# Zaggy1024/RaytracerCore

Measured on AMD Instinct MI355X. Metric: Mrays/sec (primary+secondary) and samples/sec at 1080p, Cornell box, higher is better.
Workload: dtype f32; 1 GPU; bounce.txt camera 0 1920x1080 x 256 spp per GPU per step; traversal=brute, recursion=10, kernel_build=scene-specialised (hiprtc)

## Files before the change

### raytracercore_amd/csrc/kernels_path.hip

```cpp
#include "../../include/rtcore_rng.h"
#include "rt_kernels.h"
#ifdef RT_SCENE_CONST
#include "rt_scene_const.h"
#endif

namespace rtc {
namespace {

struct V3 {
    float x, y, z;
};
__device__ __forceinline__ V3 v3(float x, float y, float z) { return V3{x, y, z}; }
__device__ __forceinline__ V3 xyz(float4 a) { return V3{a.x, a.y, a.z}; }
__device__ __forceinline__ V3 operator+(V3 a, V3 b) { return {a.x + b.x, a.y + b.y, a.z + b.z}; }
__device__ __forceinline__ V3 operator-(V3 a, V3 b) { return {a.x - b.x, a.y - b.y, a.z - b.z}; }
__device__ __forceinline__ V3 operator*(V3 a, float s) { return {a.x * s, a.y * s, a.z * s}; }
__device__ __forceinline__ V3 operator*(V3 a, V3 b) { return {a.x * b.x, a.y * b.y, a.z * b.z}; }
__device__ __forceinline__ V3 operator-(V3 a) { return {-a.x, -a.y, -a.z}; }
__device__ __forceinline__ float dot(V3 a, V3 b) { return fmaf(a.x, b.x, fmaf(a.y, b.y, a.z * b.z)); }
__device__ __forceinline__ bool known_zero(float c)
{
#if defined(RT_SCENE_CONST)
    return __builtin_constant_p(c) && c == 0.0f;
#else
// ... 815 lines not shown
            col = xyz(M.specular) + xyz(M.diffuse) + emis;
            return 1;
        }
        if (S.bounce >= s.recursion) {
            rec->type = RT_BOUNCE_RECURSION_COMPLETE;
            col = S.tint * emis;
            return 1;
        }
    }

    const float shin = M.shininess;
    float z = 1.0f, sz = 0.0f;
    if (!(s.facts & FACT_INF_SHININESS) || !(__builtin_isinf(shin) && shin > 0.0f)) {
        const float a = __builtin_amdgcn_logf(next_u(S.rng)) * M.inv_shininess;
        z = __builtin_amdgcn_exp2f(a);
        sz = fsqrt(one_minus_exp2_2a<!SLOT>(a, z));
    }
    const Frame fr = make_frame(nrm);
    const V3 rough = horizon(fr, nrm, z, sz, next_u(S.rng));

    const float diff_lum = M.diffuse.w, emis_lum = M.emission.w;
    float spec_lum = M.specular.w, refr_lum = M.refraction.w;
    const float cs = -dot(rough, S.d);
    if constexpr (REC) rec->cos_in = cs;
    float cos_out = 0.0f, ior_ratio = 0.0f;
    const bool some_lum = SLOT ? ((refr_lum > 0.0f) | (spec_lum > 0.0f))
                               : ((__float_as_int(refr_lum) > 0) | (__float_as_int(spec_lum) > 0));
    if ((s.facts & FACT_IOR) && some_lum && M.ior != 0.0f &&
        cs >= 0.0f) {
        ior_ratio = inside ? M.eta_exit : M.eta_enter;
        const float sin_out = ior_ratio * fsqrt(1.0f - cs * cs);
        if (sin_out >= 1.0f) {
            refr_lum = 0.0f;
            if constexpr (REC) rec->fresnel = 1.0f;
        } else {
            cos_out = fsqrt(1.0f - sin_out * sin_out);
            const float ra = fmaf(-ior_ratio, cos_out, cs), rb = fmaf(ior_ratio, cos_out, cs);
            const float pa = fmaf(ior_ratio, cs, -cos_out), pb = fmaf(ior_ratio, cs, cos_out);
            const float ratio = (ra * ra * pb * pb + pa * pa * rb * rb) * rcp(rb * rb * pb * pb) * 0.5f;
            spec_lum *= ratio;
            refr_lum *= 1.0f - ratio;
            if constexpr (REC) rec->fresnel = ratio;
        }
    } else {
        refr_lum = 0.0f;
    }
    const float total = diff_lum + spec_lum + refr_lum + emis_lum;
    if (total <= 0.0f) {
        if constexpr (REC) rec->type = RT_BOUNCE_PURE_BLACK;
        col = S.tint * emis;
        return 1;
    }
    float ray_rand = next_u(S.rng) * total;
    const bool transmit = refr_lum != 0.0f && (ray_rand -= refr_lum) <= 0.0f;
    const bool specular = !transmit && spec_lum != 0.0f && (ray_rand -= spec_lum) <= 0.0f;
    const bool diffuse = !transmit && !specular && diff_lum != 0.0f && (ray_rand -= diff_lum) <= 0.0f;
    if (!(transmit | specular | diffuse)) {
        if constexpr (REC) rec->type = RT_BOUNCE_EMISSION;
        col = S.tint * emis;
        return 1;
    }
    if constexpr (REC) rec->type = transmit ? RT_BOUNCE_TRANSMITTED : specular ? RT_BOUNCE_SPECULAR : RT_BOUNCE_DIFFUSE;
    V3 out_dir, new_tint;
    if (diffuse) {
        const float dz = acos_turn2(next_u(S.rng));
        const float ds = fsqrt(fmaxf(0.0f, 1.0f - dz * dz));
        out_dir = horizon(fr, nrm, dz, ds, next_u(S.rng));
        new_tint = xyz(M.diffuse);
    } else {
        const float al = transmit ? ior_ratio : 1.0f;
        const float be = transmit ? cs * ior_ratio - cos_out : 2.0f * cs;
        out_dir = madd(rough, be, S.d * al);
        if (specular && !(dot(out_dir, nrm) > 0.0f)) {
            if constexpr (REC) rec->type = RT_BOUNCE_SPECULAR_FAIL;
            col = S.tint * emis;
            return 1;
        }
        new_tint = transmit ? (inside ? v3(1.0f, 1.0f, 1.0f) : xyz(M.refraction)) : xyz(M.specular);
    }
    S.o = pos;
    S.d = out_dir * (renormalise_at<SLOT>(s, S.bounce + 1) ? fmaf(-0.5f, dot(out_dir, out_dir), 1.5f) : 1.0f);
    S.prev = b.sg >> 1;
    if (VN && s.n_vn > 0 && kind == RT_PRIM_TRIANGLE && (fl & F_HASNORMALS)) {
        bool gin2;
        if (!__builtin_isnan(S.d.x + S.d.y + S.d.z) && vn_rehit_test(prims_d[id], (double)bu, (double)bv, S.d, gin2) &&
            ((fl & F_TWOSIDED) || !(gin2 ^ ((fl & F_INVERT) != 0)))) {
            const bool front = dot(out_dir, nrm) > 0.0f;
            if (front ? (gin2 == gin) : (gin2 != gin))
                S.prev = -2 - ((b.sg & ~1) | (int)gin2);
        }
    }
    S.tint = S.tint * (new_tint * (SLOT ? fmaxf(total, 1.0f) : vmax1(total)));
    S.bounce++;
    return 0;
}

#ifndef RT_PATH_WAVES
#define RT_PATH_WAVES 7
#endif
#ifndef RT_GROUPED_WAVES
#define RT_GROUPED_WAVES 7
#endif
#ifndef RT_WIDE_STACK
#define RT_WIDE_STACK 16
#endif
#ifndef RT_SPEC_PRIMS
#define RT_SPEC_PRIMS 2
#endif
#ifndef RT_BVH_WAVES
#define RT_BVH_WAVES 7
#endif
#ifndef RT_BVH2_WAVES
#define RT_BVH2_WAVES 6
#endif

struct ShadeRecs {
    const PrimF* prims;
    const MatF* mats;
    const XformF* xfs;
};
template <bool LDS, class SceneT>
__device__ __forceinline__ ShadeRecs stage_scene(const SceneT& s, const PrimF* prims_g, const MatF* mats_g,
                                                 const XformF* xf, float4* lds_scene)
{
    if (!LDS) return ShadeRecs{prims_g, mats_g, xf};
    const int n_p = s.n_slots * (int)(sizeof(PrimF) / 16), n_m = s.n_mats * (int)(sizeof(MatF) / 16),
              n_x = s.n_xf * (int)(sizeof(XformF) / 16);
    const float4* gp = reinterpret_cast<const float4*>(prims_g);
    const float4* gm = reinterpret_cast<const float4*>(mats_g);
    const float4* gx = reinterpret_cast<const float4*>(xf);
    for (int i = threadIdx.x; i < n_p; i += blockDim.x) lds_scene[i] = gp[i];
    for (int i = threadIdx.x; i < n_m; i += blockDim.x) lds_scene[n_p + i] = gm[i];
    for (int i = threadIdx.x; i < n_x; i += blockDim.x) lds_scene[n_p + n_m + i] = gx[i];
    __syncthreads();
    return ShadeRecs{reinterpret_cast<const PrimF*>(lds_scene), reinterpret_cast<const MatF*>(lds_scene + n_p),
                     reinterpret_cast<const XformF*>(lds_scene + n_p + n_m)};
}

__device__ __forceinline__ int scene_lds_float4s(const PathScene& s)
{
    return s.n_slots * (int)(sizeof(PrimF) / 16) + s.n_mats * (int)(sizeof(MatF) / 16) +
           s.n_xf * (int)(sizeof(XformF) / 16);
}

struct Lane {
    bool active, item_open, live;
    unsigned item;
    int fx, fy, s_next;
    rt_key2 pkey;
    float ar, ag, ab;
    unsigned cnt;
    unsigned pool_next, pool_end;
    unsigned split_j;
};

__device__ __forceinline__ void lane_init(Lane& L)
{
    L.active = true;
    L.item_open = L.live = false;
    L.item = 0;
    L.fx = L.fy = L.s_next = 0;
    L.pkey = rt_key2{0u, 0u};
    L.ar = L.ag = L.ab = 0.0f;
    L.cnt = 0;
    L.pool_next = L.pool_end = 0;
    L.split_j = 0;
}

__device__ __forceinline__ unsigned lanes_below(unsigned long long m)
{
    return __builtin_amdgcn_mbcnt_hi((unsigned)(m >> 32), __builtin_amdgcn_mbcnt_lo((unsigned)m, 0u));
}
template <bool TABLE = false, class ParT>
__device__ __forceinline__ void item_pixel(unsigned item, const ParT& p, int& px, int& py, int& c, int& fx, int& fy)
{
    const unsigned q = item & 63u, t = item >> 6;
    c = (int)(t & (unsigned)(p.n_chunks - 1));
    unsigned by, bx;
    const unsigned blk = t >> p.log2_chunks;
    if (TABLE && p.cull != nullptr) {
        const unsigned v = p.cull[kCullTable + blk];
        bx = v & 0xFFFFu;
        by = v >> 16;
    } else if (p.magic_bx != 0) {
        by = __umulhi(blk, p.magic_bx);
        bx = blk - by * (unsigned)p.blocks_x;
    } else {
        divmod(blk, (unsigned)p.blocks_x, p.inv_blocks_x, by, bx);
    }
    px = (int)bx * 8 + (int)(q & 7);
    py = (int)by * 8 + (int)(q >> 3);
    fx = p.x0 + px;
    fy = p.y0 + py;
    if (p.band > 0) {
        unsigned bq, br;
        if (p.band_log2 >= 0) {
            bq = (unsigned)py >> p.band_log2;
            br = (unsigned)py & (unsigned)(p.band - 1);
        } else {
            divmod((unsigned)py, (unsigned)p.band, p.inv_band, bq, br);
        }
        fy = p.y0 + ((int)bq * p.band_stride + p.band_offset) * p.band + (int)br;
    }
}

struct QueryRay {
    V3 o, d;
    bool valid;
};
__device__ __forceinline__ QueryRay load_query_ray(const double2* __restrict__ rays, unsigned i)
{
    const double2 r0 = rays[4 * (size_t)i], r1 = rays[4 * (size_t)i + 1], r2 = rays[4 * (size_t)i + 2],
                  r3 = rays[4 * (size_t)i + 3];
    QueryRay q;
    q.o = v3((float)r0.x, (float)r0.y, (float)r1.x);
    q.d = v3((float)r2.x, (float)r2.y, (float)r3.x);
    const float inf = __builtin_huge_valf();
    const bool finite = (fabsf(q.o.x) < inf) & (fabsf(q.o.y) < inf) & (fabsf(q.o.z) < inf) & (fabsf(q.d.x) < inf) &
                        (fabsf(q.d.y) < inf) & (fabsf(q.d.z) < inf) & (fabs(r1.y) < __builtin_huge_val()) &
                        (fabs(r3.y) < __builtin_huge_val());
    q.valid = finite & ((q.d.x != 0.0f) | (q.d.y != 0.0f) | (q.d.z != 0.0f));
    return q;
}

template <class ParT>
__device__ __forceinline__ unsigned item_ray(unsigned item, const ParT& p)
{
    return ((item >> (6 + p.log2_chunks)) << 6) | (item & 63u);
}

template <class ParT>
__device__ __forceinline__ void list_pixel(unsigned pix, const ParT& p, int& fx, int& fy)
{
    unsigned q, r;
    divmod(pix, (unsigned)p.scene.width, p.inv_frame_w, q, r);
    fx = (int)r;
    fy = (int)q;
}

template <bool NT, class ParT>
__device__ __forceinline__ int item_sample(const Lane& L, const ParT& p)
{
    if (!NT) return L.s_next;
    const int c = (int)((L.item >> 6) & (unsigned)(p.n_chunks - 1));
    return c * p.chunk + (int)(L.cnt & 0xFFu) + (int)((L.cnt >> 8) & 0xFFu);
}
template <bool NT, int SRC, bool ROWS, class ParT, class CamT>
__device__ __forceinline__ bool start_rows_on(const ParT& p, [[maybe_unused]] const CamT& cam)
{
    if constexpr (NT || SRC != ITEMS_TILE || !ROWS) {
        return false;
    } else {
#ifdef RT_SCENE_CONST
        if (!cam_frustum(cam) || cam_dof(cam)) return false;
#endif
        return p.starts != nullptr;
    }
}
typedef float row_f4 __attribute__((ext_vector_type(4)));
#ifdef __HIP_DEVICE_COMPILE__
typedef __attribute__((address_space(1))) row_f4 row_g4;
typedef __attribute__((address_space(1))) unsigned char row_g1;
#else
typedef row_f4 row_g4;
typedef unsigned char row_g1;
#endif
template <class ParT>
__device__ __forceinline__ unsigned start_row_offset(const ParT& p, unsigned r, int lane)
{
    const unsigned wave = blockIdx.x * 4u + (unsigned)__builtin_amdgcn_readfirstlane((int)(threadIdx.x >> 6));
    return (((wave * (unsigned)p.start_rows + r) << 6) | (unsigned)lane) * 16u;
}

template <bool NT, int SRC = ITEMS_TILE, bool ROWS = false, class ParT, class SceneT, class CamT>
__device__ __forceinline__ void refill(Lane& L, Sample& S, const ParT& p, const SceneT& s, const CamT& cam, int lane,
                                      unsigned total)
{
    const bool need = L.active && !L.live && (!L.item_open || L.cnt < 65536u);
    if (need && L.item_open) {
        const float4 part = make_float4(L.ar, L.ag, L.ab, __uint_as_float((L.cnt & 0xFFu) | ((L.cnt & 0xFF00u) << 8)));
        if (NT) {
            typedef float nt_f4 __attribute__((ext_vector_type(4)));
            const nt_f4 v = {part.x, part.y, part.z, part.w};
            __builtin_nontemporal_store(v, reinterpret_cast<nt_f4*>(&p.partial[L.item]));
        } else {
            p.partial[L.item] = part;
        }
        L.item_open = false;
        L.ar = L.ag = L.ab = 0.0f;
    }
    const unsigned long long m = __ballot(need);
    if (m) {
        unsigned k = (unsigned)__popcll(m);
        const unsigned avail = L.pool_end - L.pool_next;
        unsigned fresh = 0, fresh_len = (unsigned)p.pool;
        bool draw = k > avail;
        if (!NT && draw && k < (unsigned)p.batch && __ballot(L.active && !need) != 0ull) {
            draw = false;
            k = avail;
        }
        if (draw) {
            const bool linear = p.linear != 0;
            unsigned got = linear ? total : (unsigned)p.n_split << 28;
            if (lane == 0) {
                if (p.n_split <= 1) {
                    const unsigned f = atomicAdd(p.counter, 1u);
                    if (f < p.split_tickets[0]) got = linear ? f * (unsigned)p.pool : f;
                } else {
                    const unsigned g0 = blockIdx.x & (unsigned)(p.n_split - 1);
                    for (; L.split_j < (unsigned)p.n_split; L.split_j++) {
                        const unsigned g = (g0 + L.split_j) & (unsigned)(p.n_split - 1);
                        const unsigned f = atomicAdd(p.counter + kSplitStride * g, 1u);
                        if (f < p.split_tickets[g]) {
                            got = linear ? p.split_start[g] + f * (unsigned)p.pool : f | g << 28;
                            break;
                        }
                    }
                }
            }
            got = __builtin_amdgcn_readfirstlane(got);
            fresh = linear ? got : total;
            if (!linear && (got >> 28) < (unsigned)p.n_split)
                ticket_items(p, got >> 28, got & 0xFFFFFFFu, fresh, fresh_len);
        }
        if (need) {
            const unsigned r = NT ? lanes_below(m) : (unsigned)__popcll(m & ((1ull << lane) - 1ull));
            L.item = r < avail ? L.pool_next + r : fresh + (r - avail);
            if (r >= k) {
            } else if (L.item >= total) {
                L.active = false;
            } else if constexpr (SRC == ITEMS_PIXELS) {
                const unsigned li = item_ray(L.item, p);
                const int s0 = (int)((L.item >> 6) & (unsigned)(p.n_chunks - 1)) * p.chunk;
                if (li < p.n_rays && s0 < p.spp) {
                    const unsigned pix = p.pixel_list[li];
                    if (pix < p.n_frame_px) {
                        L.item_open = true;
                        if (!NT) L.s_next = s0;
                        L.cnt = (unsigned)(min(p.spp, s0 + p.chunk) - s0) << 16;
                        if (!NT) {
                            list_pixel(pix, p, L.fx, L.fy);
                            if (p.pkeys) L.pkey = p.pkeys[pix];
                            else L.pkey = rt_rng_pixel_key(p.seed_key, (unsigned long long)pix);
                        }
                    }
                }
            } else if constexpr (SRC == ITEMS_RAYS) {
                const unsigned ri = item_ray(L.item, p);
                const int s0 = (int)((L.item >> 6) & (unsigned)(p.n_chunks - 1)) * p.chunk;
                if (ri < p.n_rays && s0 < p.spp) {
                    L.item_open = true;
                    if (!NT) L.s_next = s0;
                    L.cnt = (unsigned)(min(p.spp, s0 + p.chunk) - s0) << 16;
                    if (!NT) {
                        L.fx = (int)ri;
                        L.pkey = rt_rng_pixel_key(p.seed_key, p.stream_base + (unsigned long long)ri);
                    }
                }
            } else {
                int px, py, c, fx, fy;
                item_pixel<!NT>(L.item, p, px, py, c, fx, fy);
                if (px < p.w && py < p.h && c * p.chunk < p.spp) {
                    L.item_open = true;
                    const int s0 = c * p.chunk;
                    if (!NT) L.s_next = s0;
                    L.cnt = (unsigned)(min(p.spp, s0 + p.chunk) - s0) << 16;
                    if (!NT) {
                        L.fx = fx;
                        L.fy = fy;
                    }
                    const unsigned long long pix = (unsigned long long)fy * (unsigned long long)p.scene.width +
                                                   (unsigned long long)fx;
                    if (!NT && p.pkeys) L.pkey = p.pkeys[pix];
                    else if (!NT) L.pkey = rt_rng_pixel_key(p.seed_key, pix);
                }
            }
        }
        if (draw) {
            L.pool_next = fresh + (k - avail);
            L.pool_end = fresh + fresh_len;
        } else {
            L.pool_next += k;
        }
        if (k != 0 && start_rows_on<NT, SRC, ROWS>(p, cam)) {
            const unsigned n = need && L.item_open ? L.cnt >> 16 : 0u;
            row_g1* const rows = (row_g1*)(unsigned long long)p.starts;
            for (unsigned j = 0; j < (unsigned)p.start_rows; j++) {
                if (j < n) {
                    S.rng = rt_rng_from_pixel_key(L.pkey, p.sample_base + (unsigned long long)(L.s_next + (int)j));
                    float sx, sy;
                    sample_point<true>(L.fx, L.fy, S, sx, sy);
                    S.d = camera_ray(cam, sx, sy).d;
                    const row_f4 v = {S.d.x, S.d.y, S.d.z, __uint_as_float(S.rng.x)};
                    *(row_g4*)(rows + start_row_offset(p, j, lane)) = v;
                }
            }
        }
    }
    if constexpr (SRC == ITEMS_RAYS) {
        if (L.active && L.item_open && !L.live && L.cnt >= 65536u) {
            const unsigned ri = NT ? item_ray(L.item, p) : (unsigned)L.fx;
            if (NT) L.pkey = rt_rng_pixel_key(p.seed_key, p.stream_base + (unsigned long long)ri);
            const QueryRay q = load_query_ray(p.ray_list, ri);
            if (q.valid) {
                S.rng = rt_rng_from_pixel_key(L.pkey, p.sample_base + (unsigned long long)item_sample<NT>(L, p));
                (void)rt_rng_next24(&S.rng);
                (void)rt_rng_next24(&S.rng);
                S.o = q.o;
                S.d = q.d;
                S.tint = v3(1.0f, 1.0f, 1.0f);
                S.bounce = 0;
                S.prev = -1;
                L.live = true;
            } else {
                const unsigned left = L.cnt >> 16;
                L.cnt = (L.cnt & 0xFFFFu) + (left << 8);
                if (!NT) L.s_next += (int)left;
            }
        }
        return;
    }
    if (L.active && L.item_open && !L.live && L.cnt >= 65536u) {
        if (start_rows_on<NT, SRC, ROWS>(p, cam)) {
            const unsigned r = (L.cnt & 0xFFu) + ((L.cnt >> 8) & 0xFFu);
            const row_g1* const rows = (const row_g1*)(unsigned long long)p.starts;
            const row_f4 v = *(const row_g4*)(rows + start_row_offset(p, r, lane));
            const V3 d = v3(v.x, v.y, v.z);
            S.rng.x = __float_as_uint(v.w);
            S.o = madd(d, cam.image_plane, xyz(cam.position));
            S.d = d;
            S.tint = v3(1.0f, 1.0f, 1.0f);
            S.bounce = 0;
            S.prev = -1;
            L.live = true;
            return;
        }
        int fx = L.fx, fy = L.fy;
        if (NT && SRC == ITEMS_PIXELS) {
            const unsigned pix = p.pixel_list[item_ray(L.item, p)];
            list_pixel(pix, p, fx, fy);
            L.pkey = rt_rng_pixel_key(p.seed_key, (unsigned long long)pix);
        } else if (NT) {
            int px, py, c;
            item_pixel(L.item, p, px, py, c, fx, fy);
            L.pkey = rt_rng_pixel_key(p.seed_key, (unsigned long long)fy * (unsigned long long)p.scene.width +
                                                      (unsigned long long)fx);
        }
        S.rng = rt_rng_from_pixel_key(L.pkey, p.sample_base + (unsigned long long)item_sample<NT>(L, p));
        start_sample<!NT>(cam, fx, fy, S);
        L.live = true;
    }
}

template <bool VN, bool PIN = false, bool SLOT = false, bool REC = false, class SceneT, class VnP, class TestP, class ParT>
__device__ __forceinline__ void bounce(Lane& L, Sample& S, const SceneT& s, const ShadeRecs& R, VnP vnormals, TestP tests,
                                       const PrimD* prims_d, const Best& b, [[maybe_unused]] const ParT& p)
{
    V3 col;
    [[maybe_unused]] BounceRec rec;
    [[maybe_unused]] const V3 ro = S.o, rd = S.d, rtint = S.tint;
    [[maybe_unused]] const int rbounce = S.bounce;
    [[maybe_unused]] unsigned rsample = 0;
    if constexpr (REC) {
        if (p.rec_rays) {
            int px, py, c, fx, fy;
            item_pixel(L.item, p, px, py, c, fx, fy);
            rsample = ((unsigned)py * (unsigned)p.w + (unsigned)px) * (unsigned)p.spp + (unsigned)item_sample<SLOT>(L, p);
        }
    }
    const int r = shade<VN, PIN, SLOT, REC>(s, R.prims, R.mats, R.xfs, vnormals, tests, prims_d, b, S, col, &rec);
    if constexpr (REC) {
        const unsigned slot = rsample * (unsigned)(s.recursion + 1) + (unsigned)rbounce;
        if (p.rec_rays && slot < p.rec_max && rbounce <= s.recursion) {
            float4* q = p.rec_rays + (size_t)kRecRows * slot;
            q[0] = make_float4(__int_as_float(rec.prim_id), __int_as_float(rec.type), __int_as_float(rec.inside), rec.distance);
            q[1] = make_float4(rec.fresnel, rec.cos_in, __int_as_float(rbounce), 0.0f);
            q[2] = make_float4(rec.pos.x, rec.pos.y, rec.pos.z, rec.nrm.x);
            q[3] = make_float4(rec.nrm.y, rec.nrm.z, ro.x, ro.y);
            q[4] = make_float4(ro.z, rd.x, rd.y, rd.z);
            q[5] = make_float4(rtint.x, rtint.y, rtint.z, 0.0f);
            if (r != 0)
                p.rec_samples[rsample] = r == 1 ? make_float4(0.0f + col.x, 0.0f + col.y, 0.0f + col.z, __int_as_float(rbounce + 1))
                                                : make_float4(-1.0f, -1.0f, -1.0f, __int_as_float(rbounce + 1));
        }
    }
    if (r != 0) {
        const bool hit = r == 1;
        L.ar += hit ? col.x : 0.0f;
        L.ag += hit ? col.y : 0.0f;
        L.ab += hit ? col.z : 0.0f;
        L.cnt += hit ? 1u - 65536u : 256u - 65536u;
        if (!SLOT) L.s_next++;
        L.live = false;
        if (!SLOT) {
            asm volatile("" : "=v"(S.o.x), "=v"(S.o.y), "=v"(S.o.z), "=v"(S.d.x), "=v"(S.d.y), "=v"(S.d.z),
                         "=v"(S.tint.x), "=v"(S.tint.y), "=v"(S.tint.z), "=v"(S.bounce), "=v"(S.prev),
                         "=v"(S.rng.x));
        }
    }
}

template <bool STATS, class ParT>
__device__ __forceinline__ void flush_counts(unsigned long long wave_rays, const Counters& cnt, const ParT& p,
                                             int lane)
{
    if (lane == 0) atomicAdd(p.rays, wave_rays);
    if (STATS) {
        unsigned long long a = cnt.nodes, t = cnt.tris, q = cnt.sphs;
        for (int off = 32; off > 0; off >>= 1) {
            a += __shfl_down(a, off);
            t += __shfl_down(t, off);
            q += __shfl_down(q, off);
        }
        if (lane == 0) {
            atomicAdd(p.stats + 0, a);
            atomicAdd(p.stats + 1, t);
            atomicAdd(p.stats + 2, q);
            atomicAdd(p.stats + 3, cnt.cyc_start);
            atomicAdd(p.stats + 4, cnt.cyc_trace);
            atomicAdd(p.stats + 5, cnt.cyc_shade);
            atomicAdd(p.stats + 6, cnt.iters);
        }
        unsigned long long mx = cnt.max_steps, ov = cnt.ovf_pushes, ms = cnt.max_sp, ot = cnt.outer;
        for (int off = 32; off > 0; off >>= 1) {
            mx = max(mx, (unsigned long long)__shfl_down(mx, off));
            ov += __shfl_down(ov, off);
            ms = max(ms, (unsigned long long)__shfl_down(ms, off));
            ot += __shfl_down(ot, off);
        }
        if (lane == 0) {
            atomicMax(p.stats + 7, mx);
            atomicAdd(p.stats + 8, ov);
            atomicMax(p.stats + 9, ms);
            atomicAdd(p.stats + 10, ot);
        }
    }
}

#ifdef __HIP_DEVICE_COMPILE__
#define RT_AS_CONST __attribute__((address_space(4)))
#else
#define RT_AS_CONST
#endif
typedef RT_AS_CONST const CameraF CameraC;
typedef RT_AS_CONST const PathParams ParamsC;

template <bool CULL, bool LDS, bool STATS, bool VN, int SRC = ITEMS_TILE>
__device__ __forceinline__ void path_body(const CameraF* __restrict__ camp, const PathParams* __restrict__ pp)
{
    const ParamsC& P0 = *(const ParamsC*)pp;
    extern __shared__ float4 lds_scene[];
    const ShadeRecs R = stage_scene<LDS>(P0.scene, P0.prims, P0.mats, P0.xf, lds_scene);
    const int lane = threadIdx.x & 63;
    const unsigned total = (unsigned)P0.n_chunks * (unsigned)P0.n_pad;
    Lane L;
    lane_init(L);
    Sample S;
    S.prev = -1;
    S.bounce = 0;
    Counters cnt{};
    unsigned long long wave_rays = 0;
    const unsigned long long bound_off = P0.scene_bound != 0 ? 0ull : ~0ull;

    while (true) {
        unsigned long long t0 = 0, t1 = 0, t2 = 0;
        if (STATS) t0 = __builtin_readcyclecounter();
        const CameraC* cp = (const CameraC*)camp;
        asm volatile("" : "+s"(cp));
        const ParamsC* pq = (const ParamsC*)pp;
        asm volatile("" : "+s"(pq));
#ifdef RT_SCENE_CONST
        const PathScene& sc = *(const PathScene*)kSceneW;
#else
        const auto& sc = pq->scene;
#endif
#if defined(RT_SCENE_CONST) && RT_SCENE_CONST_CAMERA
        refill<false, ITEMS_TILE, !STATS && !VN>(L, S, *pq, sc, *(const CameraF*)kCameraW, lane, total);
#else
        refill<false, SRC, !STATS && !VN>(L, S, *pq, sc, *cp, lane, total);
#endif
        if (!__any(L.active)) break;
        if (STATS) t1 = __builtin_readcyclecounter();
        wave_rays += (unsigned)__popcll(__ballot(L.live));
        if (L.live) {
#ifdef RT_SCENE_CONST
            const auto tests = (const TestRec*)kTestsW;
            const auto rects = (const RectRec*)kRectsW;
            const auto frames = (const FrameRec*)kFramesW;
            const auto boxes = (const BoxRec*)kFramesW;
            const auto groups = (const GroupRec*)kGroupsW;
            const auto xf = (const XformF*)kXfW;
#else
            const auto tests = (const RT_AS_CONST TestRec*)pq->tests;
            const auto rects = (const RT_AS_CONST RectRec*)pq->rects;
            const auto frames = (const RT_AS_CONST FrameRec*)pq->frames;
            const auto boxes = (const RT_AS_CONST BoxRec*)pq->frames;
            const auto groups = (const RT_AS_CONST GroupRec*)pq->groups;
            const auto xf = (const RT_AS_CONST XformF*)pq->xf;
#endif
            const auto vnormals = (const RT_AS_CONST float4*)pq->vnormals;
            Best b = query_start<VN>(sc, S.prev);
            bool query = true;
            if (!STATS && (!CULL || RT_BOUND_GROUPED) &&
                __builtin_expect((__ballot(L.live && S.bounce != 0) | bound_off) == 0ull, 0))
                query = __any(L.live && scene_meets(sc, S.o, S.d));
            if (query)
                trace_brute<CULL, STATS>(sc, groups, tests, rects, frames, boxes, xf, S.o, S.d, S.prev, b, cnt.tris,
                                         cnt.sphs, cnt.nodes);
            test_planes(sc, tests, S.o, S.d, S.prev, b);
            if (VN && __builtin_isnan(S.d.x + S.d.y + S.d.z)) b = Best{__builtin_huge_valf(), -1};
            if (STATS) t2 = __builtin_readcyclecounter();
            bounce<VN, false, false, STATS>(L, S, sc, R, vnormals, tests, pq->prims_d, b, *pq);
        } else if (STATS) {
            t2 = __builtin_readcyclecounter();
        }
        if (STATS) {
            const unsigned long long t3 = __builtin_readcyclecounter();
            cnt.cyc_start += t1 - t0;
            cnt.cyc_trace += t2 - t1;
            cnt.cyc_shade += t3 - t2;
            cnt.iters++;
        }
    }
    if (!STATS && SRC == ITEMS_TILE && P0.cull != nullptr && blockIdx.x == 0 && threadIdx.x < 64)
        wave_rays += ((unsigned long long)P0.cull[0] | (unsigned long long)P0.cull[1] << 32) * (unsigned long long)P0.spp;
    flush_counts<STATS>(wave_rays, cnt, *(const ParamsC*)pp, lane);
}

template <bool CULL, bool LDS, bool STATS, bool VN, int SRC = ITEMS_TILE>
__global__ void __launch_bounds__(256, CULL ? RT_GROUPED_WAVES : RT_PATH_WAVES)
    path_kernel(PathScene, const CameraF* __restrict__ camp, const PathParams* __restrict__ pp, const TestRec*,
                const RectRec*, const FrameRec*, const PrimF*, const NodeF*, const Node4Q*, const GroupRec*,
                const XformF*, const MatF*, const float4*)
{
    path_body<CULL, LDS, STATS, VN, SRC>(camp, pp);
}

template <bool STATS, class GroupP, class RectP, class BoxP>
__device__ __forceinline__ void test_outer(GroupP groups, RectP rects, BoxP boxes, V3 o, V3 d, int prev, Best& b,
                                           unsigned& n_tests)
{
    const V3 id = v3(slab_rcp_lean(d.x), slab_rcp_lean(d.y), slab_rcp_lean(d.z));
    const V3 oi = o * id;
    const GroupRec G = groups[0];
    if (STATS) n_tests += G.n_rect[0] + G.n_rect[1] + G.n_rect[2] + G.n_flat_extra;
    RectP r = rects + __float_as_int(G.lo.w);
    rect_group<0>(r, G.n_rect[0], o, d, id, oi, prev, b);
    r += G.n_rect[0];
    rect_group<1>(r, G.n_rect[1], o, d, id, oi, prev, b);
    r += G.n_rect[1];
    rect_group<2>(r, G.n_rect[2], o, d, id, oi, prev, b);
    for (int j = G.frame_first + G.n_frames; j < G.frame_first + G.n_frames + G.n_boxes; j++) {
        const BoxRec B = boxes[j];
        hit_box<false>(B, o, d, id, oi, prev, b);
    }
}

template <bool STATS, class TestP, class RowP, class XfP>
__device__ __forceinline__ void test_leaf(TestP tests, RowP rows, XfP xf, int pend, V3 o, V3 d, int prev, Best& b,
                                          unsigned& n_tri, unsigned& n_sph)
{
    int k, kend;
    uint32_t lfl;
    leaf_decode(pend, k, kend, lfl);
    float4 r[RT_SPEC_PRIMS][3];
    uint32_t fl[RT_SPEC_PRIMS];
#pragma unroll
    for (int j = 0; j < RT_SPEC_PRIMS; j++) {
        r[j][0] = rows[3 * (k + j)];
        r[j][1] = rows[3 * (k + j) + 1];
        r[j][2] = rows[3 * (k + j) + 2];
    }
    if (lfl == kLeafGeneric) {
#pragma unroll
        for (int j = 0; j < RT_SPEC_PRIMS; j++) fl[j] = __float_as_uint(tests[k + j].meta.y);
    } else {
#pragma unroll
        for (int j = 0; j < RT_SPEC_PRIMS; j++) fl[j] = lfl;
    }
#pragma unroll
    for (int j = 0; j < RT_SPEC_PRIMS; j++) {
        pin4(r[j][0]);
        pin4(r[j][1]);
        pin4(r[j][2]);
    }
#pragma unroll
    for (int j = 0; j < RT_SPEC_PRIMS; j++) {
        if (j == 0 || k + j < kend) {
            const bool sph = (fl[j] & KIND_MASK) == RT_PRIM_SPHERE;
            if (STATS) {
                if (sph) n_sph++;
                else n_tri++;
            }
            if (sph) hit_sph_rows(r[j][0], r[j][1], fl[j], k + j, k + j, o, d, prev, xf, b);
            else hit_tri_rows(r[j][0], r[j][1], r[j][2], fl[j], k + j, k + j, o, d, prev, b);
        }
    }
}

struct Walk {
    bool more;
    int ref;
    int sp;
    int pend;
};
__device__ __forceinline__ void walk_start(Walk& w, int root, bool tree)
{
    w.ref = root;
    w.sp = 0;
    w.pend = -1;
    w.more = tree;
    if (root < 0) {
        w.pend = ~root;
        w.more = false;
    }
}
struct WalkStep {
    bool ended;
    bool leaf_step, can_node;
    int sp_visit;
};
template <int STACK, bool ANY, bool STATS = false, int WIDTH = 4, class FetchT, class TestP, class RowP, class XfP>
__device__ __forceinline__ WalkStep walk_step(Walk& w, bool trav, int spec, FetchT fetch, V3 id, V3 oi, const TravStack& stk,
                                              TestP tests, RowP rows, XfP xf, V3 o, V3 d, int prev, Best& b,
                                              unsigned& n_tri, unsigned& n_sph)
{
    WalkStep st;
    st.can_node = trav && w.more && w.ref >= 0;
    const bool blocked = trav && w.pend >= 0 && !st.can_node;
    st.leaf_step = __ballot(st.can_node) == 0 || __popcll(__ballot(blocked)) >= spec;
    st.ended = false;
    st.sp_visit = w.sp;
// ... 1119 lines not shown
```

### raytracercore_amd/csrc/launch_params.cpp

```cpp
#include "launch_params.h"

#include <algorithm>
#include <cmath>
#include <cstdlib>

#include "host_scene.h"

namespace rtc {

void set_item_order(PathParams& p)
{
    const char* e = getenv("RTCORE_ITEM_ORDER");
    bool dense = !(e && e[0] == '0');
    const unsigned slots = (unsigned)p.pool / 64u;
    const unsigned used = (unsigned)((p.spp + p.chunk - 1) / p.chunk);
    const unsigned n_blocks = (unsigned)(p.n_pad / 64);
    for (;; dense = false) {
        const unsigned n_real = dense ? used : (unsigned)p.n_chunks;
        const unsigned n_full = dense && p.spp % p.chunk != 0 ? used - 1 : n_real;
        p.tpb = n_full / slots;
        p.tail_first = p.tpb * (unsigned)p.pool;
        p.tail_len = (n_real - p.tpb * slots) * 64u;
        p.magic_tpb = 0;
        if (p.tpb <= 1) break;
        const uint64_t M = ((1ull << 32) + p.tpb - 1) / p.tpb;
        const uint64_t err = M * p.tpb - (1ull << 32);
        if (M < (1ull << 32) && (uint64_t)n_blocks * p.tpb * err < (1ull << 32)) {
            p.magic_tpb = (unsigned)M;
            break;
        }
    }
    p.linear = p.tail_len == 0 && p.tpb * slots == (unsigned)p.n_chunks;
    for (int g = 0; g < kMaxSplit; g++) {
        const unsigned b = g < p.n_split ? (p.split_start[g + 1] - p.split_start[g]) >> (p.log2_chunks + 6) : 0u;
        p.split_full[g] = b * p.tpb;
        p.split_tickets[g] = p.split_full[g] + (p.tail_len ? b : 0u);
    }
}

void set_blocks(PathParams& p, int n_blocks)
{
    p.n_pad = n_blocks * 64;
    p.n_split = 1;
    int want = kMaxSplit;
    if (const char* e = getenv("RTCORE_XCD_SPLIT")) want = atoi(e) > 0 ? kMaxSplit : 1;
    if (want > 1 && n_blocks >= 4 * kMaxSplit) p.n_split = kMaxSplit;
    for (int g = 0; g <= p.n_split; g++)
        p.split_start[g] = (unsigned)((int64_t)n_blocks * g / p.n_split) * (unsigned)(p.n_chunks * 64);
    set_item_order(p);
}

PathParams make_params_for(int kernel, int chunks_over, int pool_over, int x0, int y0, int w, int h, int spp,
                           uint64_t seed, uint64_t base, double chunk_npix)
{
    PathParams p{};
    p.x0 = x0;
    p.y0 = y0;
    p.w = w;
    p.h = h;
    p.band = 0;
    p.spp = spp;
    const int base_chunks = kernel >= 2 ? 64 : 24;
    int chunks = base_chunks;
    const double npix = chunk_npix > 0.0 ? chunk_npix : (double)w * (double)h;
    if (npix > 0 && npix < 2073600.0)
        chunks = (int)std::min(8.0 * base_chunks, base_chunks * std::ceil(2073600.0 / npix));
    else if (npix > 2073600.0)
        chunks = (int)std::max(base_chunks / 4.0, std::ceil(base_chunks * 2073600.0 / npix));
    if (const char* e = getenv("RTCORE_PATH_CHUNKS")) chunks = std::max(1, atoi(e));
    if (chunks_over > 0) chunks = chunks_over;
    p.chunk = std::max(1, std::min(64, (spp + chunks - 1) / chunks));
    const int used = (spp + p.chunk - 1) / p.chunk;
    p.log2_chunks = 0;
    while ((1 << p.log2_chunks) < used) p.log2_chunks++;
    p.n_chunks = 1 << p.log2_chunks;
    p.blocks_x = (w + 7) / 8;
    p.n_pad = p.blocks_x * ((h + 7) / 8) * 64;
    p.inv_blocks_x = 1.0f / (float)p.blocks_x;
    p.magic_bx = 0;
    if (p.blocks_x > 1 && !getenv("RTCORE_NO_MAGIC_DIV")) {
        const uint64_t M = ((1ull << 32) + (uint64_t)p.blocks_x - 1) / (uint64_t)p.blocks_x;
        const uint64_t err = M * (uint64_t)p.blocks_x - (1ull << 32);
        const uint64_t max_blk = (uint64_t)(p.n_pad / 64);
        if (M < (1ull << 32) && max_blk * err < (1ull << 32)) p.magic_bx = (unsigned)M;
    }
    int pool_mul = kernel == 0 ? 1 : 2;
    if (const char* e = getenv("RTCORE_POOL_MUL")) pool_mul = std::max(1, std::min(64, atoi(e)));
    if (pool_over > 0) pool_mul = std::max(1, std::min(64, pool_over / 64));
    p.pool = 64;
    while (p.pool < 64 * pool_mul && p.pool < 64 * p.n_chunks) p.pool *= 2;
    p.batch = kernel < 2 ? 64 : 0;
    if (const char* e = getenv("RTCORE_ITEM_BATCH")) p.batch = std::max(0, std::min(64, atoi(e)));
    p.scene_bound = 1;
    if (const char* e = getenv("RTCORE_SCENE_BOUND")) p.scene_bound = atoi(e) != 0 ? 1 : 0;
    p.refill = 28;
    if (const char* e = getenv("RTCORE_BVH_REFILL")) p.refill = std::max(1, std::min(64, atoi(e)));
    p.spec = 12;
    if (const char* e = getenv("RTCORE_BVH_SPEC")) p.spec = std::max(1, std::min(64, atoi(e)));
    set_blocks(p, p.n_pad / 64);
    p.seed = seed;
    p.seed_key = rt_rng_seed_key(seed);
    p.sample_base = base;
    return p;
}

PathParams make_params_rays(int kernel, int64_t n, int spp, uint64_t seed, uint64_t base, uint64_t stream_base)
{
    PathParams p = make_params_for(kernel, 0, 0, 0, 0, 8, (int)((n + 7) / 8), spp, seed, base, 2073600.0);
    p.n_rays = (unsigned)n;
    p.stream_base = stream_base;
    return p;
}

PathParams make_params_pixels(int kernel, int64_t n, int spp, uint64_t seed, uint64_t base, int width, int height)
{
    PathParams p = make_params_for(kernel, 0, 0, 0, 0, 8, (int)((n + 7) / 8), spp, seed, base, 2073600.0);
    p.n_rays = (unsigned)n;
    p.n_frame_px = (unsigned)((uint64_t)width * (uint64_t)height);
    p.inv_frame_w = 1.0f / (float)width;
    return p;
}

int64_t render_rays_max_n(int kernel, int spp)
{
    const PathParams p = make_params_for(kernel, 0, 0, 0, 0, 8, 8, spp, 0, 0, 2073600.0);
    const int64_t blocks = (int64_t)(0xF0000000ull / ((uint64_t)p.n_chunks * 64u));
    return std::min<int64_t>(blocks * 64, (int64_t)1 << 30);
}

StartRowsPlan plan_start_rows(int kernel, bool instrumented, bool vertex_normals, int camera_kind, bool dof, int chunk,
                              int grid_blocks)
{
    const StartRowsPlan off{false, 0, 0};
    if (kernel < 0 || kernel >= 2 || instrumented || vertex_normals || camera_kind != RT_CAMERA_FRUSTUM || dof) return off;
    if (chunk < 1 || chunk > kStartRowsMaxChunk || grid_blocks < 1) return off;
    if (const char* e = getenv("RTCORE_START_ROWS"))
        if (atoi(e) == 0) return off;
    const size_t bytes = (size_t)grid_blocks * 4u * (size_t)chunk * 64u * 16u;
    if (bytes > kStartRowsCap) return off;
    return StartRowsPlan{true, chunk, bytes};
}

void set_band(PathParams& p, int band, int stride, int offset)
{
    p.band = band;
    p.band_stride = stride;
    p.band_offset = offset;
    p.band_log2 = -1;
    for (int k = 0; k < 31; k++)
        if (band == (1 << k)) p.band_log2 = k;
    p.inv_band = 1.0f / (float)band;
}

int band_set_rows(int H, int band, int stride, int offset)
{
    int rows = 0;
    for (int b = offset; b * band < H; b += stride) rows += std::min(band, H - b * band);
    return rows;
}

int band_slot_rows(int H, int band, int stride)
{
    int m = 0;
    for (int o = 0; o < stride; o++) m = std::max(m, band_set_rows(H, band, stride, o));
    return m;
}

void scatter_band_set(const unsigned char* slot, size_t plane, int W, int H, int band, int stride, int offset,
                      rt_color* sum_rgb, uint32_t* samples, uint32_t* misses)
{
    const double* hs = reinterpret_cast<const double*>(slot);
    const uint32_t* hn = reinterpret_cast<const uint32_t*>(hs + 3 * plane);
    const uint32_t* hm = hn + plane;
    parallel_ranges((size_t)W, 64, [&](size_t xa, size_t xb) {
        int tr = 0;
        for (int b = offset; b * band < H; b += stride)
            for (int y = b * band; y < std::min(H, (b + 1) * band); y++, tr++)
                for (size_t x = xa; x < xb; x++) {
                    const size_t i = (size_t)tr * W + x, o = x * H + y;
                    sum_rgb[o].r += hs[i];
                    sum_rgb[o].g += hs[plane + i];
                    sum_rgb[o].b += hs[2 * plane + i];
                    samples[o] += hn[i];
                    misses[o] += hm[i];
                }
    });
}

int64_t list_tickets(const PathParams& p, uint32_t* out, int64_t cap_words)
{
    int64_t n = 0;
    for (int g = 0; g < p.n_split; g++)
        for (unsigned t = 0; t < p.split_tickets[g]; t++, n++) {
            unsigned first = 0, len = 0;
            ticket_items(p, (unsigned)g, t, first, len);
            if (3 * (n + 1) <= cap_words) {
                out[3 * n] = (uint32_t)g;
                out[3 * n + 1] = first;
                out[3 * n + 2] = len;
            }
        }
    return n;
}

}
```

### raytracercore_amd/csrc/rt_kernels.h

```cpp
#pragma once
#include "../../include/rtcore_rng.h"
#include "rt_internal.h"

namespace rtc {

constexpr int kMaxSplit = 8;
constexpr int kSplitStride = 32;

enum ItemSource : int { ITEMS_TILE = 0, ITEMS_RAYS = 1, ITEMS_PIXELS = 2 };

struct PathParams {
    int x0, y0, w, h;
    int band, band_stride, band_offset;
    int band_log2;
    float inv_band;
    int spp;
    int chunk;
    int n_chunks;
    int log2_chunks;
    int blocks_x;
    int n_pad;
    int refill;
    int spec;
    int pool;
    float inv_blocks_x;
    unsigned magic_bx;
    unsigned long long seed;
    rt_key2 seed_key;
    unsigned long long sample_base;
    const rt_key2* pkeys;
    unsigned int* counter;
    int n_split;
    unsigned split_start[9];
    unsigned tpb;
    unsigned magic_tpb;
    unsigned tail_first;
    unsigned tail_len;
    int linear;
    int batch;
    unsigned split_full[8];
    unsigned split_tickets[8];
    float4* partial;
    unsigned long long* rays;
    int* stack_ovf;
    unsigned long long* stats;
    PathScene scene;
    const TestRec* tests;
    const float4* rows;
    const RectRec* rects;
    const FrameRec* frames;
    const PrimF* prims;
    const GroupRec* groups;
    const NodeF* nodes;
    const Node4Q* nodes4;
    const XformF* xf;
    const MatF* mats;
    const float4* vnormals;
    const PrimD* prims_d;
    float4* ray_log;
    unsigned int* ray_log_n;
    unsigned int ray_log_cap;
    float4* rec_rays;
    float4* rec_samples;
    unsigned int rec_max;
    union {
        const double2* ray_list;
        const uint32_t* pixel_list;
        float4* starts;
    };
    unsigned int n_rays;
    int start_rows;
    union {
        unsigned long long stream_base;
        struct {
            unsigned int n_frame_px;
            float inv_frame_w;
        };
    };
    int scene_bound;
    const unsigned int* cull;
};
static_assert(__builtin_offsetof(PathParams, start_rows) == __builtin_offsetof(PathParams, n_rays) + 4 &&
                  __builtin_offsetof(PathParams, scene_bound) == __builtin_offsetof(PathParams, n_rays) + 16,
              "start_rows takes the padding after n_rays");
constexpr int kCullTable = 4;
constexpr int kRecRows = 6;

template <class ParT>
__host__ __device__ inline void ticket_items(const ParT& p, unsigned g, unsigned t, unsigned& first, unsigned& len)
{
    const unsigned full = p.split_full[g];
    unsigned blk, off;
    if (t < full) {
        blk = p.magic_tpb ? (unsigned)(((unsigned long long)t * p.magic_tpb) >> 32) : t;
        off = (t - blk * p.tpb) * (unsigned)p.pool;
        len = (unsigned)p.pool;
    } else {
        blk = t - full;
        off = p.tail_first;
        len = p.tail_len;
    }
    first = p.split_start[g] + (blk << (p.log2_chunks + 6)) + off;
}

struct TraceRaysParams {
    const float4* rays;
    float2* hits;
    unsigned int n;
    unsigned int* counter;
    int* stack_ovf;
    const TestRec* tests;
    const float4* rows;
    const Node4Q* nodes4;
    const XformF* xf;
    int root4;
    int spec;
    const GroupRec* outer;
    const RectRec* outer_rects;
    const FrameRec* outer_boxes;
    unsigned long long* stats;
};

#ifndef __HIPCC_RTC__
struct QueryParams {
    const double2* rays;
    float4* hits;
    unsigned int n;
    unsigned int* counter;
    int* stack_ovf;
    PathScene scene;
    const TestRec* tests;
    const float4* rows;
    const RectRec* rects;
    const FrameRec* frames;
    const PrimF* prims;
    const GroupRec* groups;
    const Node4Q* nodes4;
    const XformF* xf;
    const float4* vnormals;
    int root4;
    int n_nodes4;
    int spec;
};
constexpr int kHitRows = 3;

int query_blocks_per_cu(int kernel);
hipError_t launch_query(const QueryParams& p, int kernel, int grid_blocks, hipStream_t stream);
hipError_t launch_query_exact(const DevScene& s, const rt_ray* d_rays, unsigned n, rt_hit* d_hits, hipStream_t stream);
struct OccludedParams {
    QueryParams q;
    const double* t_max;
    unsigned char* out;
    int early;
};
int occluded_blocks_per_cu(int kernel);
hipError_t launch_occluded(const OccludedParams& p, int kernel, int grid_blocks, hipStream_t stream);
hipError_t launch_occluded_exact(const DevScene& s, const rt_ray* d_rays, const double* d_t_max, unsigned n,
                                 unsigned char* d_out, hipStream_t stream);
void fill_launch(const DevScene& s, int variant, PathParams& p);

hipError_t launch_primary_ids(const DevScene& s, const CameraD& cam, int x0, int y0, int w, int h, int mode,
                              int32_t* d_ids, hipStream_t stream);

hipError_t launch_select_pixels(const DevScene& s, const CameraD& cam, const rt_select_item* d_items, int n_items, int x0,
                                int y0, int w, int h, rt_selection* d_out, hipStream_t stream);
hipError_t launch_select_rays(const DevScene& s, const rt_select_item* d_items, int n_items, const rt_ray* d_rays,
                              unsigned n, rt_selection* d_out, hipStream_t stream);

int path_variant(int kernel, bool lds);
constexpr int kStackOverflow = 44;
constexpr int kTestSpares = 3;
int path_wide_stack();
size_t path_lds_bytes(const DevScene& s);
size_t path_dyn_lds(const DevScene& s, int variant);
hipError_t launch_path(const DevScene& s, const CameraF* d_cam, const PathParams* d_params, int variant,
                       int grid_blocks, hipStream_t stream, bool stats, ItemSource src = ITEMS_TILE);
int path_blocks_per_cu(int variant, size_t dyn_lds, bool stats, bool vn, ItemSource src = ITEMS_TILE);
int trace_rays_blocks_per_cu(int waves);
int debug_vn_rehit(const double v0[3], const double e01[3], const double e02[3], int mirror, double u, double v,
                   const float dir[3], int* inside, double* t, double o[3]);
hipError_t launch_trace_rays(const TraceRaysParams& p, int waves, int grid_blocks, hipStream_t stream);
hipError_t launch_pixel_keys(rt_key2 seed_key, int w, int h, rt_key2* out, hipStream_t stream);
hipError_t compact_leaves(const TestRec* d_tests, int n_records, float4* d_rows, NodeF* d_nodes, int n_nodes,
                          Node4Q* d_nodes4, int n_nodes4, bool rewrite, hipStream_t stream);

hipError_t launch_accumulate(const PathParams& p, double* d_sum, uint32_t* d_samples, uint32_t* d_misses,
                             hipStream_t stream, size_t plane = 0);
hipError_t launch_tonemap(int w, int h, const double* d_sum, const uint32_t* d_samples, const uint32_t* d_misses,
                          rt_color back, double back_alpha, double exposure, int32_t* d_argb, hipStream_t stream);
struct TileRec {
    double r, g, b;
    uint32_t samples, misses;
};
hipError_t launch_accumulate_rays(const PathParams& p, double* d_sum, uint32_t* d_samples, uint32_t* d_misses,
                                  TileRec* d_recs, hipStream_t stream);
hipError_t launch_accumulate_pixels(const PathParams& p, double* d_sum, uint32_t* d_samples, uint32_t* d_misses,
                                    double* d_q, uint32_t* d_batches, size_t plane, hipStream_t stream);
struct PixelRec {
    double r, g, b, q;
    uint32_t samples, misses, batches, pad;
};
hipError_t launch_accumulate_pixels_recs(const PathParams& p, PixelRec* d_recs, hipStream_t stream);
hipError_t launch_tile_host_layout(int w, int h, const double* d_sum, const uint32_t* d_samples,
                                  const uint32_t* d_misses, TileRec* d_out, hipStream_t stream);
hipError_t launch_trace_host_layout(int w, int h, int spp, int recursion, const float4* d_rays, const float4* d_samples,
                                    float4* d_rays_out, float4* d_samples_out, hipStream_t stream);
hipError_t launch_colors_1spp(const PathParams& p, float* d_out, hipStream_t stream);

#endif

}
```

Before: 123,100 Mrays/s.

## Gate per-wave sample starts into rounds when tickets run long

Adds a 'sample rounds' mode to the brute-force tile path-tracing refill. Once a ticket's rays-per-sample ratio shows paths running deep, a lane starts its next sample only after the whole wave has no live paths. The aim is to keep lanes in lockstep on bounce depth and cut divergence from mixing fresh primary rays with deep secondary bounces. The trade-off is idle lanes while waiting for the slowest path in each round. The mode is on by default through an adaptive heuristic and can be overridden with RTCORE_SAMPLE_ROUNDS.

```diff
diff --git a/raytracercore_amd/csrc/kernels_path.hip b/raytracercore_amd/csrc/kernels_path.hip
--- a/raytracercore_amd/csrc/kernels_path.hip
+++ b/raytracercore_amd/csrc/kernels_path.hip
@@ -991,6 +991,8 @@
     unsigned cnt;
     unsigned pool_next, pool_end;
     unsigned split_j;
+    bool rounds;
+    unsigned ticket_mark;
 };
 
 __device__ __forceinline__ void lane_init(Lane& L)
@@ -1004,6 +1006,8 @@
     L.cnt = 0;
     L.pool_next = L.pool_end = 0;
     L.split_j = 0;
+    L.rounds = false;
+    L.ticket_mark = 0;
 }
 
 __device__ __forceinline__ unsigned lanes_below(unsigned long long m)
@@ -1111,10 +1115,13 @@
     return (((wave * (unsigned)p.start_rows + r) << 6) | (unsigned)lane) * 16u;
 }
 
-template <bool NT, int SRC = ITEMS_TILE, bool ROWS = false, class ParT, class SceneT, class CamT>
+template <bool NT, int SRC = ITEMS_TILE, bool ROWS = false, bool ROUNDS = false, class ParT, class SceneT, class CamT>
 __device__ __forceinline__ void refill(Lane& L, Sample& S, const ParT& p, const SceneT& s, const CamT& cam, int lane,
-                                      unsigned total)
-{
+                                      unsigned total, [[maybe_unused]] unsigned rays_now = 0)
+{
+    static_assert(!ROUNDS || (!NT && SRC == ITEMS_TILE), "sample rounds: the brute-force tile instances");
+    bool go = true;
+    if constexpr (ROUNDS) go = !L.rounds || __ballot(L.live) == 0ull;
     const bool need = L.active && !L.live && (!L.item_open || L.cnt < 65536u);
     if (need && L.item_open) {
         const float4 part = make_float4(L.ar, L.ag, L.ab, __uint_as_float((L.cnt & 0xFFu) | ((L.cnt & 0xFF00u) << 8)));
@@ -1158,6 +1165,11 @@
                 }
             }
             got = __builtin_amdgcn_readfirstlane(got);
+            if constexpr (ROUNDS) {
+                L.rounds = __builtin_amdgcn_readfirstlane(
+                               (int)ticket_rounds(p, s.recursion, L.pool_end == 0u, rays_now - L.ticket_mark)) != 0;
+                L.ticket_mark = rays_now;
+            }
             fresh = linear ? got : total;
             if (!linear && (got >> 28) < (unsigned)p.n_split)
                 ticket_items(p, got >> 28, got & 0xFFFFFFFu, fresh, fresh_len);
@@ -1259,7 +1271,7 @@
         }
         return;
     }
-    if (L.active && L.item_open && !L.live && L.cnt >= 65536u) {
+    if (go && L.active && L.item_open && !L.live && L.cnt >= 65536u) {
         if (start_rows_on<NT, SRC, ROWS>(p, cam)) {
             const unsigned r = (L.cnt & 0xFFu) + ((L.cnt >> 8) & 0xFFu);
             const row_g1* const rows = (const row_g1*)(unsigned long long)p.starts;
@@ -1414,9 +1426,11 @@
         const auto& sc = pq->scene;
 #endif
 #if defined(RT_SCENE_CONST) && RT_SCENE_CONST_CAMERA
-        refill<false, ITEMS_TILE, !STATS && !VN>(L, S, *pq, sc, *(const CameraF*)kCameraW, lane, total);
+        refill<false, ITEMS_TILE, !STATS && !VN, !STATS && !VN>(L, S, *pq, sc, *(const CameraF*)kCameraW, lane, total,
+                                                         (unsigned)wave_rays);
 #else
-        refill<false, SRC, !STATS && !VN>(L, S, *pq, sc, *cp, lane, total);
+        refill<false, SRC, !STATS && !VN, !STATS && !VN && SRC == ITEMS_TILE>(L, S, *pq, sc, *cp, lane, total,
+                                                                              (unsigned)wave_rays);
 #endif
         if (!__any(L.active)) break;
         if (STATS) t1 = __builtin_readcyclecounter();
diff --git a/raytracercore_amd/csrc/launch_params.cpp b/raytracercore_amd/csrc/launch_params.cpp
--- a/raytracercore_amd/csrc/launch_params.cpp
+++ b/raytracercore_amd/csrc/launch_params.cpp
@@ -93,6 +93,8 @@
     if (const char* e = getenv("RTCORE_ITEM_BATCH")) p.batch = std::max(0, std::min(64, atoi(e)));
     p.scene_bound = 1;
     if (const char* e = getenv("RTCORE_SCENE_BOUND")) p.scene_bound = atoi(e) != 0 ? 1 : 0;
+    p.sample_rounds = 1;
+    if (const char* e = getenv("RTCORE_SAMPLE_ROUNDS")) p.sample_rounds = std::max(0, std::min(2, atoi(e)));
     p.refill = 28;
     if (const char* e = getenv("RTCORE_BVH_REFILL")) p.refill = std::max(1, std::min(64, atoi(e)));
     p.spec = 12;
diff --git a/raytracercore_amd/csrc/rt_kernels.h b/raytracercore_amd/csrc/rt_kernels.h
--- a/raytracercore_amd/csrc/rt_kernels.h
+++ b/raytracercore_amd/csrc/rt_kernels.h
@@ -78,11 +78,15 @@
         };
     };
     int scene_bound;
+    int sample_rounds;
     const unsigned int* cull;
 };
 static_assert(__builtin_offsetof(PathParams, start_rows) == __builtin_offsetof(PathParams, n_rays) + 4 &&
                   __builtin_offsetof(PathParams, scene_bound) == __builtin_offsetof(PathParams, n_rays) + 16,
               "start_rows takes the padding after n_rays");
+static_assert(__builtin_offsetof(PathParams, sample_rounds) == __builtin_offsetof(PathParams, scene_bound) + 4 &&
+                  __builtin_offsetof(PathParams, cull) == __builtin_offsetof(PathParams, scene_bound) + 8,
+              "sample_rounds takes the padding after scene_bound");
 constexpr int kCullTable = 4;
 constexpr int kRecRows = 6;
 
@@ -101,6 +105,16 @@
         len = p.tail_len;
     }
     first = p.split_start[g] + (blk << (p.log2_chunks + 6)) + off;
+}
+
+constexpr unsigned kRoundsNum = 4, kRoundsDen = 5;
+template <class ParT>
+__host__ __device__ inline bool ticket_rounds(const ParT& p, int recursion, bool first, unsigned prev_rays)
+{
+    if (p.sample_rounds != 1) return p.sample_rounds == 2;
+    if (first) return false;
+    const unsigned long long samples = (unsigned long long)(unsigned)p.pool * (unsigned long long)(unsigned)p.chunk;
+    return (unsigned long long)prev_rays * kRoundsDen >= samples * (unsigned long long)(unsigned)(recursion + 1) * kRoundsNum;
 }
 
 struct TraceRaysParams {
```

Measured after the change: 132,000 Mrays/s, median of 6. +7.3%, better.
